# alevar/tiebrush

Measured on AMD Instinct MI355X. Metric: input alignment records/sec collapsed (tiebrush) + bases/sec covered (tiecov), higher is better.
Workload: dtype int64; 1 GPU; c3: 64 synthetic sorted BAMs x 5000000 100bp reads per GPU, --clip collapse + tiecov -c -j of the result; records_per_gpu=320000000, groups_out=25086541, parallelism=files-per-rank x1, ranks_seen=1, resident=SoA in HBM before the timed region, contexts=3

## Files before the change

### tiebrush_amd/csrc/collapse.hip

```cpp
#include <stdlib.h>

#include <chrono>

#include "cb_tiles.hpp"
#include "dev_common.hpp"
#include "rx_w64.hpp"
#include "scan_op.hpp"
#include "strategy.hpp"
#include "tbk_internal.h"
#include "wgroup.h"

namespace {

struct EffKey {
  uint32_t khi_h, khi_l;
  int32_t kend;
  uint32_t flag_cnt;
};
struct EffOp {
  __device__ __forceinline__ EffKey operator()(const EffKey& a, const EffKey& b) const {
    uint64_t ak = ((uint64_t)a.khi_h << 32) | a.khi_l, bk = ((uint64_t)b.khi_h << 32) | b.khi_l;
    bool take_b = (b.flag_cnt >> 31) || bk > ak || (bk == ak && b.kend > a.kend);
    EffKey r;
    r.khi_h = take_b ? b.khi_h : a.khi_h;
// ... 353 lines not shown
__global__ void col_recgroup_w_k(uint32_t n, const uint32_t* __restrict__ rec_sg, const uint32_t* __restrict__ ginv, int32_t* __restrict__ rec_group) {
  uint32_t i = blockIdx.x * blockDim.x + threadIdx.x;
  if (i >= n) return;
  const uint32_t sg = rec_sg[i];
  rec_group[i] = sg == 0xFFFFFFFFu ? -1 : (int32_t)ginv[sg];
}


constexpr uint32_t YS_NT = 1024;
constexpr uint32_t YS_NL = 128;
struct YsIn {
  uint32_t ng;
  const uint32_t* gperm;
  const uint32_t* ns;
  const uint32_t* gpoff;
  const uint16_t* pfile;
  const uint64_t* ghi;
  const uint64_t* gfmask;
};
__device__ __forceinline__ uint64_t ys_spread32(uint64_t x) {
  x = (x | (x << 16)) & 0x0000FFFF0000FFFFull;
  x = (x | (x << 8)) & 0x00FF00FF00FF00FFull;
  x = (x | (x << 4)) & 0x0F0F0F0F0F0F0F0Full;
  x = (x | (x << 2)) & 0x3333333333333333ull;
  x = (x | (x << 1)) & 0x5555555555555555ull;
  return x;
}
__device__ __forceinline__ void ys_mask_from_files(uint64_t files, uint32_t c, uint64_t* lo, uint64_t* hi) {
  const uint64_t a = ys_spread32(files & 0xFFFFFFFFull), b = ys_spread32(files >> 32);
  *lo = c == 0u ? a : (c == 1u ? a << 1 : (a | (a << 1)));
  *hi = c == 0u ? b : (c == 1u ? b << 1 : (b | (b << 1)));
}
__device__ __forceinline__ uint64_t wave_bit_transpose(uint64_t x) {
  const uint32_t lane = lane_id();
#define YS_TSTEP(J, M)                                                                     \
  {                                                                                        \
    const uint64_t tt = ((uint64_t)(uint32_t)__shfl_xor((int)(uint32_t)(x >> 32), J, 64) << 32) | (uint32_t)__shfl_xor((int)(uint32_t)x, J, 64); \
    x = (lane & J) ? (((tt >> J) & M) | (x & ~M)) : ((x & M) | ((tt & M) << J));           \
  }
  YS_TSTEP(32, 0x00000000FFFFFFFFull)
  YS_TSTEP(16, 0x0000FFFF0000FFFFull)
  YS_TSTEP(8, 0x00FF00FF00FF00FFull)
  YS_TSTEP(4, 0x0F0F0F0F0F0F0F0Full)
  YS_TSTEP(2, 0x3333333333333333ull)
  YS_TSTEP(1, 0x5555555555555555ull)
#undef YS_TSTEP
  return x;
}
struct YsAgg {
  uint32_t first_tid, last_tid;
  int32_t mx;
  uint32_t whole;
};
__device__ __forceinline__ YsAgg ys_combine(const YsAgg& a, const YsAgg& b) {
  if (b.last_tid == 0u) return a;
  if (a.last_tid == 0u) return b;
  YsAgg r;
  r.first_tid = a.first_tid;
  r.last_tid = b.last_tid;
  const bool joins = b.whole && b.first_tid == a.last_tid;
  r.mx = joins ? (a.mx > b.mx ? a.mx : b.mx) : b.mx;
  r.whole = joins ? a.whole : 0u;
  return r;
}
struct YsCells {
  uint32_t (*a)[YS_NL];
  uint32_t (*b)[YS_NL];
  int32_t (*m)[YS_NL];
  __device__ __forceinline__ YsAgg get(uint32_t x, uint32_t c) const { return YsAgg{a[x][c] & 0x7FFFFFFFu, b[x][c], m[x][c], a[x][c] >> 31}; }
  __device__ __forceinline__ void put(uint32_t x, uint32_t c, const YsAgg& v) const {
    a[x][c] = v.first_tid | (v.whole << 31);
    b[x][c] = v.last_tid;
    m[x][c] = v.mx;
  }
};
__device__ __forceinline__ YsAgg ys_chain_cells(const YsCells& P, uint32_t c, YsAgg run) {
  for (uint32_t x = 0; x < YS_NT / 64; ++x) {
    const YsAgg mine = P.get(x, c);
    P.put(x, c, run);
    run = ys_combine(run, mine);
  }
  return run;
}
__global__ __launch_bounds__(YS_NT) void yd_lcount_k(YsIn S, const uint4* __restrict__ gpk , uint32_t ntiles,
                                                     uint32_t* __restrict__ table , uint4* __restrict__ agg ,
                                                     uint64_t* __restrict__ gwb ) {
  __shared__ uint64_t wb[YS_NT / 64][YS_NL];
  __shared__ uint32_t g_tid[YS_NT];
  __shared__ int32_t g_e1[YS_NT];
  __shared__ uint32_t pa[YS_NT / 64][YS_NL], pb[YS_NT / 64][YS_NL];
  __shared__ int32_t pm[YS_NT / 64][YS_NL];
  const YsCells P{pa, pb, pm};
  uint64_t lo = 0, hi = 0;
  {
    const uint32_t o = blockIdx.x * YS_NT + threadIdx.x;
    if (o < S.ng) {
      const uint32_t sg = S.gperm[o];
      const uint32_t c = (uint32_t)S.ghi[sg] & 3u;
      const uint32_t n = S.gfmask ? 0u : S.ns[sg], p0 = S.gfmask ? 0u : S.gpoff[sg];
      uint64_t files = 0;
      if (S.gfmask)
        files = S.gfmask[sg];
      else
        for (uint32_t i = 0; i < n; ++i) files |= 1ull << S.pfile[p0 + i];
      ys_mask_from_files(files, c, &lo, &hi);
      const uint4 g = gpk[o];
      g_tid[threadIdx.x] = g.x;
      g_e1[threadIdx.x] = (int32_t)g.z + 1;
    }
  }
  {
    const uint32_t x = threadIdx.x >> 6, l = lane_id();
    const uint64_t a = wave_bit_transpose(lo), b = wave_bit_transpose(hi);
    wb[x][l] = a;
    wb[x][64u + l] = b;
    uint64_t* out = gwb + (size_t)blockIdx.x * (YS_NT / 64) * YS_NL + x * YS_NL;
    out[l] = a;
    out[64u + l] = b;
  }
  __syncthreads();
  for (uint32_t q = threadIdx.x; q < (YS_NT / 64) * YS_NL; q += YS_NT) {
    const uint32_t x = q / YS_NL, c = q % YS_NL;
    YsAgg A{0u, 0u, INT32_MIN, 1u};
    for (uint64_t m = wb[x][c]; m; m &= m - 1) {
      const uint32_t g = x * 64u + (uint32_t)__builtin_ctzll(m);
      A = ys_combine(A, YsAgg{g_tid[g], g_tid[g], g_e1[g], 1u});
    }
    P.put(x, c, A);
  }
  __syncthreads();
  if (threadIdx.x < YS_NL) {
    const uint32_t c = threadIdx.x;
    uint32_t n = 0;
    YsAgg A{0u, 0u, INT32_MIN, 1u};
    for (uint32_t x = 0; x < YS_NT / 64; ++x) {
      n += (uint32_t)__builtin_popcountll(wb[x][c]);
      A = ys_combine(A, P.get(x, c));
    }
    table[(size_t)c * ntiles + blockIdx.x] = n;
    agg[(size_t)c * ntiles + blockIdx.x] = make_uint4(A.first_tid, A.last_tid, (uint32_t)A.mx, A.whole);
  }
}
__global__ __launch_bounds__(256) void yd_lagg_scan_k(uint4* __restrict__ agg, uint32_t ntiles) {
  __shared__ uint4 part[256];
  uint4* row = agg + (size_t)blockIdx.x * ntiles;
  const uint32_t per = (ntiles + 255u) / 256u, i0 = threadIdx.x * per, i1 = i0 + per < ntiles ? i0 + per : ntiles;
  auto un = [](const uint4& v) { return YsAgg{v.x, v.y, (int32_t)v.z, v.w}; };
  auto pk = [](const YsAgg& a) { return make_uint4(a.first_tid, a.last_tid, (uint32_t)a.mx, a.whole); };
  YsAgg A{0u, 0u, INT32_MIN, 1u};
  for (uint32_t i = i0; i < i1; ++i) A = ys_combine(A, un(row[i]));
  part[threadIdx.x] = pk(A);
  __syncthreads();
  if (threadIdx.x == 0) {
    YsAgg run{0u, 0u, INT32_MIN, 1u};
    for (uint32_t q = 0; q < 256; ++q) {
      const YsAgg mine = un(part[q]);
      part[q] = pk(run);
      run = ys_combine(run, mine);
    }
  }
  __syncthreads();
  YsAgg run = un(part[threadIdx.x]);
  for (uint32_t i = i0; i < i1; ++i) {
    const YsAgg mine = un(row[i]);
    row[i] = pk(run);
    run = ys_combine(run, mine);
  }
}
__global__ __launch_bounds__(1024) void yd_lscan_k(uint32_t* __restrict__ table, uint32_t ntiles, uint64_t* __restrict__ totals,
                                                   unsigned long long* __restrict__ nit ) {
  __shared__ uint32_t sm[16];
  __shared__ uint32_t carry_s;
  uint32_t* row = table + (size_t)blockIdx.x * ntiles;
  constexpr uint32_t E = 8;
  if (threadIdx.x == 0) carry_s = 0;
  __syncthreads();
  for (uint32_t base = 0; base < ntiles; base += 1024 * E) {
    const uint32_t i0 = base + threadIdx.x * E;
    uint32_t v[E], s = 0;
#pragma unroll
    for (uint32_t e = 0; e < E; ++e) {
      v[e] = i0 + e < ntiles ? row[i0 + e] : 0u;
      s += v[e];
    }
    uint32_t tot;
    uint32_t ex = carry_s + block_excl_sum<uint32_t, 1024>(s, sm, &tot);
#pragma unroll
    for (uint32_t e = 0; e < E; ++e) {
      if (i0 + e < ntiles) row[i0 + e] = ex;
      ex += v[e];
    }
    __syncthreads();
    if (threadIdx.x == 0) carry_s += tot;
    __syncthreads();
  }
  if (threadIdx.x == 0) {
    totals[blockIdx.x] = carry_s;
    atomicAdd(nit, (unsigned long long)carry_s);
  }
}

struct YdWords {
  const uint64_t* w64;
// ... 43 lines not shown
    const uint32_t a = (h32 >> 20) & 0x3FFu, g = h32 & 0xFFFFFu;
    *e0 = st + a - 1u;
    *s1 = st + a + g;
    return 2u;
  }
  return 0u;
}

__global__ void yd_groups_k(ColIn I, uint32_t ng, const uint32_t* __restrict__ gperm, GroupAcc G, const uint64_t* __restrict__ shi,
                            const uint64_t* __restrict__ slo, YdGroups Q) {
  uint32_t o = blockIdx.x * blockDim.x + threadIdx.x;
  if (o >= ng) return;
  uint32_t sg = gperm[o];
  uint32_t q = G.first[sg];
  uint64_t h = shi[q], l = slo[q];
  int32_t st = (int32_t)(uint32_t)((h >> 2) & 0x7FFFFFFFull);
  const uint32_t tidp1 = (uint32_t)(h >> 33);
  const uint32_t en = (uint32_t)(st + (int32_t)(uint32_t)(l >> 32) - 1);
  uint32_t e0, s1;
  const uint32_t nk = yd_exons_from_key(l, (uint32_t)st, en, &e0, &s1);
  int nex = (int)nk;
  if (nex == 0) {
    const uint32_t r = (uint32_t)(G.rep[sg] & 0xFFFFFFFFull);
    walk_exons(I.pos[r], I.cig + I.cig_off[r], I.cig_off[r + 1] - I.cig_off[r], [](int, int) {}, &nex);
  }
  uint32_t xw = (uint32_t)nex;
  if (nk == 2u) {
    const uint32_t a = e0 - (uint32_t)st + 1u, g = s1 - e0 - 1u;
    if (a < (1u << 10) && g < (1u << 20)) xw = YD_X2 | (a << 20) | g;
  }
  Q.nex[o] = yd_nex_far(xw) ? (uint32_t)nex : 0u;
  Q.pk[o] = make_uint4(tidp1, (uint32_t)st, en, xw);
}

__global__ void yd_gexons_k(ColIn I, uint32_t ng, const uint32_t* __restrict__ gperm, GroupAcc G, const uint64_t* __restrict__ slo, YdGroups Q,
                            uint32_t* __restrict__ ex_s, uint32_t* __restrict__ ex_e) {
  uint32_t o = blockIdx.x * blockDim.x + threadIdx.x;
  if (o >= ng) return;
  const uint4 pk = Q.pk[o];
  if (!yd_nex_far(pk.w)) return;
  const uint32_t sg = gperm[o];
  uint32_t w = Q.xoff[o];
  {
    uint32_t e0, s1;
    const uint32_t nk = yd_exons_from_key(slo[G.first[sg]], pk.y, pk.z, &e0, &s1);
    if (nk) {
      ex_s[w] = pk.y;
      ex_e[w] = e0;
      if (nk == 2u) {
        ex_s[w + 1] = s1;
        ex_e[w + 1] = pk.z;
      }
      return;
    }
  }
  uint32_t r = (uint32_t)(G.rep[sg] & 0xFFFFFFFFull);
  int nex = 0;
  walk_exons(I.pos[r], I.cig + I.cig_off[r], I.cig_off[r + 1] - I.cig_off[r],
             [&](int es, int ee) {
               ex_s[w] = (uint32_t)es;
               ex_e[w] = (uint32_t)ee;
               ++w;
             },
             &nex);
}

struct YdEmit {
  YdGroups Q;
  YdItems Y;
  __device__ __forceinline__ void operator()(uint32_t t, uint64_t w) const {
    const uint32_t o = (uint32_t)w;
    const uint4 g = Q.pk[o];
    Y.pk[t] = make_uint4(g.x, g.y, g.z, Q.xoff[o]);
    Y.nex[t] = g.w;
  }
};

constexpr uint32_t YS_CAP = 15360;
constexpr uint32_t YS_NC = (YS_NT / 64) * YS_NL;
static_assert(YS_NC == 2 * YS_NT && YS_CAP >= 4 * YS_NC, "the staging array holds the cells' aggregates and counts first");
__global__ __launch_bounds__(YS_NT) void yd_lscatter_k(uint32_t ng, uint32_t ntiles, const uint32_t* __restrict__ table,
                                                       const uint64_t* __restrict__ totals, const uint4* __restrict__ agg,
                                                       const uint64_t* __restrict__ gwb , YdGroups Q,
                                                       YdItems Y, uint32_t* __restrict__ item) {
  __shared__ uint32_t off[YS_NL];
  __shared__ uint32_t pre[YS_NL + 1];
  __shared__ uint32_t lsum[YS_NL];
  __shared__ uint32_t lbase[YS_NL];
  __shared__ uint4 grec[YS_NT];
  __shared__ uint32_t stage[YS_CAP];
  const YsCells P{reinterpret_cast<uint32_t(*)[YS_NL]>(stage), reinterpret_cast<uint32_t(*)[YS_NL]>(stage + YS_NC),
                  reinterpret_cast<int32_t(*)[YS_NL]>(stage + 2 * YS_NC)};
  uint32_t(*pa)[YS_NL] = reinterpret_cast<uint32_t(*)[YS_NL]>(stage + 3 * YS_NC);
  const uint32_t t = threadIdx.x, c = t % YS_NL, x0 = t / YS_NL, x1 = x0 + YS_NT / YS_NL;
  const uint64_t* col = gwb + (size_t)blockIdx.x * YS_NC;
  const uint64_t m0 = col[t], m1 = col[YS_NT + t];
  if (t < YS_NL) lbase[t] = (uint32_t)totals[t];
  const uint32_t o = blockIdx.x * YS_NT + t;
  if (o < ng) grec[t] = Q.pk[o];
  __syncthreads();
  auto fold = [&](uint64_t m, uint32_t x) {
    pa[x][c] = (uint32_t)__builtin_popcountll(m);
    YsAgg A{0u, 0u, INT32_MIN, 1u};
    for (; m; m &= m - 1) {
      const uint4 g = grec[x * 64u + (uint32_t)__builtin_ctzll(m)];
      A = ys_combine(A, YsAgg{g.x, g.x, (int32_t)g.z + 1, 1u});
    }
    P.put(x, c, A);
  };
  fold(m0, x0);
  fold(m1, x1);
  __syncthreads();
  if (t < YS_NL) {
    const uint4 av = agg[(size_t)t * ntiles + blockIdx.x];
    (void)ys_chain_cells(P, t, YsAgg{av.x, av.y, (int32_t)av.z, av.w});
    uint32_t run = 0;
    for (uint32_t x = 0; x < YS_NT / 64; ++x) {
      const uint32_t n = pa[x][t];
      pa[x][t] = run;
      run += n;
    }
    lsum[t] = run;
  }
  __syncthreads();
  if (t < 64) {
    const uint32_t a = lsum[2 * t], b = lsum[2 * t + 1], inc = wave_incl_sum(a + b);
    const uint32_t ta = lbase[2 * t], tb = lbase[2 * t + 1], tinc = wave_incl_sum(ta + tb);
    pre[2 * t] = inc - a - b;
    pre[2 * t + 1] = inc - b;
    if (t == 63) pre[YS_NL] = inc;
    off[2 * t] = tinc - ta - tb + table[(size_t)(2 * t) * ntiles + blockIdx.x] - (inc - a - b);
    off[2 * t + 1] = tinc - tb + table[(size_t)(2 * t + 1) * ntiles + blockIdx.x] - (inc - b);
  }
  __syncthreads();
  const YsAgg A0 = P.get(x0, c), A1 = P.get(x1, c);
  const uint32_t s0 = pre[c] + pa[x0][c], s1 = pre[c] + pa[x1][c], T = pre[YS_NL];
  for (uint32_t r0 = 0; r0 < T; r0 += YS_CAP) {
    __syncthreads();
    const uint32_t r1 = r0 + YS_CAP;
    auto walk = [&](uint64_t m, uint32_t x, YsAgg A, uint32_t i) {
      if (i >= r1 || i + (uint32_t)__builtin_popcountll(m) <= r0) return;
      for (; m && i < r1; m &= m - 1, ++i) {
        const uint32_t g = x * 64u + (uint32_t)__builtin_ctzll(m);
        const uint4 v = grec[g];
        const bool head = A.last_tid == 0u || v.x != A.last_tid || (int32_t)v.y > A.mx;
        A = ys_combine(A, YsAgg{v.x, v.x, (int32_t)v.z + 1, 1u});
        if (i >= r0) stage[i - r0] = g | (c << 10) | ((uint32_t)head << 17);
      }
    };
    walk(m0, x0, A0, s0);
    walk(m1, x1, A1, s1);
    __syncthreads();
    const uint32_t n = T - r0 < YS_CAP ? T - r0 : YS_CAP;
    for (uint32_t i = t; i < n; i += YS_NT) {
      const uint32_t e = stage[i], g = e & (YS_NT - 1u), l = (e >> 10) & (YS_NL - 1u);
      const uint4 v = grec[g];
      const uint32_t pos = off[l] + r0 + i;
      Y.se[pos] = make_uint2(v.y, v.z);
      Y.nex[pos] = v.w | ((e >> 17) << 31);
      item[pos] = blockIdx.x * YS_NT + g;
    }
  }
}

struct SegMaxY {
  int32_t mx;
  uint32_t flag;
};
struct SegMaxYOp {
  __device__ __forceinline__ SegMaxY operator()(const SegMaxY& a, const SegMaxY& b) const {
    SegMaxY r;
    r.mx = b.flag ? b.mx : (a.mx > b.mx ? a.mx : b.mx);
    r.flag = a.flag | b.flag;
    return r;
  }
};
struct YdLoad {
  const uint64_t* list;
  YdItems Y;
  __device__ __forceinline__ bool list_head(uint32_t t) const {
    return t == 0 || (list[t] >> 32) != (list[t - 1] >> 32) || Y.tidp1(t) != Y.tidp1(t - 1);
  }
  __device__ __forceinline__ SegMaxY operator()(uint32_t t) const {
    SegMaxY s;
    s.mx = Y.end(t) + 1;
    s.flag = list_head(t) ? 1u : 0u;
    return s;
  }
};
struct HeadNex {
  uint32_t h, n;
};
struct HeadNexOp {
  __device__ __forceinline__ HeadNex operator()(const HeadNex& a, const HeadNex& b) const { return HeadNex{a.h + b.h, a.n + b.n}; }
};
struct YdAux {
  YdItems Y;
  __device__ __forceinline__ int2 operator()(uint32_t t) const { return make_int2(Y.start(t), (int)yd_nex_count(Y.nex[t])); }
};
struct YdHead {
  __device__ __forceinline__ HeadNex operator()(uint32_t, const SegMaxY& v, const SegMaxY&, const SegMaxY& ex, const int2& a) const {
    return HeadNex{(v.flag || a.x > ex.mx) ? 1u : 0u, (uint32_t)a.y};
  }
};
struct YdStore {
  YdItems Y;
  uint32_t *chain_first, *chain_noff;
  uint64_t* totals;
  uint32_t nit;
  __device__ __forceinline__ void operator()(uint32_t t, const SegMaxY&, const SegMaxY&, const SegMaxY&, const HeadNex& v, const HeadNex& ex,
                                             const int2&) const {
    if (v.h) {
      chain_first[ex.h] = t;
      chain_noff[ex.h] = ex.n;
    }
    if (t + 1 == nit) {
      totals[0] = ex.h + v.h;
      totals[1] = ex.n + v.n;
    }
  }
};

constexpr uint32_t YN_NT = 256, YN_ROWS = 4, YN_TILE = YN_NT * 4 * YN_ROWS;
__device__ __forceinline__ uint4 yn_load(const uint32_t* __restrict__ w, uint64_t i, uint32_t nit) {
  if (i + 3 < nit) return *reinterpret_cast<const uint4*>(w + i);
  uint4 v = make_uint4(0u, 0u, 0u, 0u);
  if (i < nit) v.x = w[i];
  if (i + 1 < nit) v.y = w[i + 1];
  if (i + 2 < nit) v.z = w[i + 2];
  return v;
}
__global__ __launch_bounds__(YN_NT) void yn_reduce_k(const uint32_t* __restrict__ w, uint32_t nit, unsigned long long* __restrict__ part) {
  __shared__ unsigned long long sm[YN_NT / 64];
  unsigned long long acc = 0;
#pragma unroll
  for (uint32_t r = 0; r < YN_ROWS; ++r) {
    const uint4 v = yn_load(w, (uint64_t)blockIdx.x * YN_TILE + ((uint64_t)r * YN_NT + threadIdx.x) * 4u, nit);
    const uint32_t h = (v.x >> 31) + (v.y >> 31) + (v.z >> 31) + (v.w >> 31);
    const uint32_t n = yd_nex_count(v.x) + yd_nex_count(v.y) + yd_nex_count(v.z) + yd_nex_count(v.w);
    acc += ((unsigned long long)h << 32) + n;
  }
  acc = wave_sum(acc);
// ... 809 lines not shown
      if (h32 == (0x80000000u | C_M)) shape = 0x80000000u;
      if ((h32 >> 30) == 3u) shape = h32;
    }
    g_key[2 * (size_t)o] = shi[q];
    g_key[2 * (size_t)o + 1] = (lo & 0xFFFFFFFF00000000ull) | shape;
  }
}
__global__ void col_recgroup_k(const uint64_t* __restrict__ pm, const uint32_t* __restrict__ val, const uint32_t* __restrict__ sgid,
                               const uint32_t* __restrict__ ginv, int32_t* __restrict__ rec_group) {
  const uint32_t m = (uint32_t)*pm;
  uint32_t q = blockIdx.x * blockDim.x + threadIdx.x;
  if (q < m) rec_group[val[q]] = (int32_t)ginv[sgid[q]];
}

__global__ void col_init_groups_k(const uint64_t* __restrict__ png, GroupAcc G, int32_t* __restrict__ g_yd) {
  const uint32_t ng = (uint32_t)*png;
  uint32_t g = blockIdx.x * blockDim.x + threadIdx.x;
  if (g >= ng) return;
  G.yc[g] = 0.0;
  G.ns[g] = 0;
  G.yxin[g] = 0;
  G.ydin[g] = 0;
  G.rep[g] = ~0ull;
  g_yd[g] = 0;
}

struct YdJob {
  ColIn I;
  uint32_t m, ng, cap;
  const uint32_t* val;
  const uint8_t* flags;
  const uint16_t* fidx;
  const uint32_t *sgid, *ginv, *gperm;
  GroupAcc G;
  const uint64_t *shi, *slo;
  int32_t* g_yd;
  int32_t* out_yd;
  bool win = false;
  uint32_t np = 0;
  const uint16_t* pfile = nullptr;
  const uint32_t *pgrp = nullptr, *gpoff = nullptr;
  const uint64_t* gfmask = nullptr;
};

}

int tbk_collapse_yd_run(tbk_ctx* ctx, void* jobp) {
  const YdJob J = *(const YdJob*)jobp;
  delete (YdJob*)jobp;
  const uint32_t B = 256;
  const uint32_t m = J.m, ng = J.ng;
  const ColIn& I = J.I;
  uint64_t* sc = ctx->d_scalars;
  TBK_HIP(hipSetDevice(ctx->device));
  const bool ph = ctx->dbg.phases;
  const auto p0 = std::chrono::steady_clock::now();
  auto p1 = p0, p2 = p0, p3 = p0;
  auto since = [](std::chrono::steady_clock::time_point a) { return std::chrono::duration<double, std::milli>(std::chrono::steady_clock::now() - a).count(); };
  TBK_HIP(hipMemsetAsync(sc, 0, 32 * sizeof(uint64_t), ctx->stream));
  {
    uint32_t *icnt = nullptr, *ioff = nullptr, *ocnt = nullptr, *ooff = nullptr;
    uint64_t nit64;
    const bool by_list = J.win && (!J.pgrp || tbk_yd_by_list(ctx, I.k));
    static_assert(YS_NL == 128, "tbk_yd_by_list (wgroup.h) knows the number of lists");
    const uint32_t ys_tiles = cdiv(ng, YS_NT);
    const YsIn S{ng, J.gperm, J.G.ns, J.gpoff, J.pfile, J.shi, J.gfmask};
    uint32_t* ys_table = nullptr;
    uint4* ys_agg = nullptr;
    uint64_t* ys_totals = nullptr;
    uint64_t* ys_wb = nullptr;
    uint32_t *yd_d = nullptr, *ys_item = nullptr;
    YdGroups Q{};
    if (by_list) {
      Q.pk = ws_alloc<uint4>(ctx, ng);
      Q.nex = ws_alloc<uint32_t>(ctx, ng);
      Q.xoff = ws_alloc<uint32_t>(ctx, ng);
      ys_table = ws_alloc<uint32_t>(ctx, (size_t)YS_NL * ys_tiles);
      ys_agg = ws_alloc<uint4>(ctx, (size_t)YS_NL * ys_tiles);
      ys_totals = ws_alloc<uint64_t>(ctx, YS_NL + 1);
      ys_wb = ws_alloc<uint64_t>(ctx, (size_t)ys_tiles * YS_NC);
      if (!Q.xoff || !ys_table || !ys_agg || !ys_totals || !ys_wb) return TBK_ENOMEM;
      TBK_LAUNCH(ctx, "yd_groups", yd_groups_k, cdiv(ng, B), B, 0, I, ng, J.gperm, J.G, J.shi, J.slo, Q);
      TBK_TRY(tbk_exscan_u32(ctx, Q.nex, Q.xoff, ng, sc + 5));
      TBK_LAUNCH(ctx, "yd_lcount", yd_lcount_k, ys_tiles, YS_NT, 0, S, Q.pk, ys_tiles, ys_table, ys_agg, ys_wb);
      TBK_LAUNCH(ctx, "yd_lscan", yd_lscan_k, YS_NL, 1024, 0, ys_table, ys_tiles, ys_totals, (unsigned long long*)(sc + 2));
      TBK_LAUNCH(ctx, "yd_lscan", yd_lagg_scan_k, YS_NL, 256, 0, ys_agg, ys_tiles);
    } else if (J.win) {
      ocnt = ws_alloc<uint32_t>(ctx, ng);
      ooff = ws_alloc<uint32_t>(ctx, ng);
      if (!ooff) return TBK_ENOMEM;
      TBK_LAUNCH(ctx, "yd_gcount", yd_gcount_w_k, cdiv(ng, B), B, 0, ng, J.gperm, J.G, J.shi, ocnt);
      TBK_TRY(tbk_exscan_u32(ctx, ocnt, ooff, ng, sc + 2));
    } else {
      icnt = ws_alloc<uint32_t>(ctx, m);
      ioff = ws_alloc<uint32_t>(ctx, m);
      if (!ioff) return TBK_ENOMEM;
      TBK_LAUNCH(ctx, "yd_count", yd_count_k, cdiv(m, B), B, 0, I, m, J.val, J.flags, J.fidx, icnt);
      TBK_TRY(tbk_exscan_u32(ctx, icnt, ioff, m, sc + 2));
    }
    TBK_HIP(hipMemcpyAsync(ctx->h_scalars, sc, 16 * sizeof(uint64_t), hipMemcpyDeviceToHost, ctx->stream));
    TBK_HIP(hipStreamSynchronize(ctx->stream));
    nit64 = ctx->h_scalars[2];
    p1 = p2 = p3 = std::chrono::steady_clock::now();
    if (nit64 >= (1ull << 32)) return TBK_E2BIG;
    const uint32_t nit = (uint32_t)nit64;
    if (nit) {
      uint64_t* iv = by_list ? nullptr : ws_alloc<uint64_t>(ctx, nit);
      uint64_t* iv2 = by_list ? nullptr : ws_alloc<uint64_t>(ctx, nit);
      uint32_t* io = by_list ? ws_alloc<uint32_t>(ctx, nit) : nullptr;
      yd_d = by_list ? ws_alloc<uint32_t>(ctx, nit) : nullptr;
      if (by_list && (!io || !yd_d)) return TBK_ENOMEM;
      ys_item = io;
      YdItems Y;
      if (by_list) {
        Y.pk = nullptr;
        Y.se = ws_alloc<uint2>(ctx, nit);
        Y.gxoff = Q.xoff;
        if (!Y.se) return TBK_ENOMEM;
      } else {
        Y.pk = ws_alloc<uint4>(ctx, nit);
      }
      Y.nex = ws_alloc<uint32_t>(ctx, nit);
      uint32_t* noff = ws_alloc<uint32_t>(ctx, nit);
      uint32_t* chain_first = ws_alloc<uint32_t>(ctx, nit);
      if (!chain_first) return TBK_ENOMEM;
      if (by_list) {
      } else if (J.win) {
        TBK_LAUNCH(ctx, "yd_fill", yd_fill_w_k, cdiv(J.np, B), B, 0, J.np, J.pfile, J.pgrp, J.gpoff, J.ginv, ooff, J.shi, iv);
      } else {
        ocnt = ws_alloc<uint32_t>(ctx, ng);
        ooff = ws_alloc<uint32_t>(ctx, ng);
        if (!ooff) return TBK_ENOMEM;
        TBK_LAUNCH(ctx, "yd_gcount", yd_gcount_k, cdiv(ng, B), B, 0, ng, m, J.gperm, J.G, ioff, icnt, ocnt);
        TBK_TRY(tbk_exscan_u32(ctx, ocnt, ooff, ng, nullptr));
        TBK_LAUNCH(ctx, "yd_fill", yd_fill_k, cdiv(m, B), B, 0, I, m, J.val, J.flags, J.fidx, J.sgid, J.ginv, ioff, ooff, J.G, iv);
      }
      if (!by_list) {
        Q.pk = ws_alloc<uint4>(ctx, ng);
        Q.nex = ws_alloc<uint32_t>(ctx, ng);
        Q.xoff = ws_alloc<uint32_t>(ctx, ng);
        if (!Q.xoff) return TBK_ENOMEM;
        TBK_LAUNCH(ctx, "yd_groups", yd_groups_k, cdiv(ng, B), B, 0, I, ng, J.gperm, J.G, J.shi, J.slo, Q);
        TBK_TRY(tbk_exscan_u32(ctx, Q.nex, Q.xoff, ng, sc + 5));
      }
      if (by_list) {
        TBK_LAUNCH(ctx, "yd_scatter", yd_lscatter_k, ys_tiles, YS_NT, 0, ng, ys_tiles, ys_table, ys_totals, ys_agg, ys_wb, Q, Y, io);
      } else {
        uint32_t bits = 1;
        while ((1ull << bits) < 2ull * I.k) ++bits;
        TBK_TRY(tbk_radix_sort_w64_emit(ctx, &iv, &iv2, nit, ((1ull << bits) - 1ull) << 32, true, YdEmit{Q, Y}, "yd_scatter"));
      }
      if (by_list) {
        const uint32_t ynb = cdiv(nit, YN_TILE);
        unsigned long long* ypart = ws_alloc<unsigned long long>(ctx, ynb);
        if (!ypart) return TBK_ENOMEM;
        TBK_LAUNCH(ctx, "yd_number", yn_reduce_k, ynb, YN_NT, 0, Y.nex, nit, ypart);
        TBK_LAUNCH(ctx, "yd_number", yn_spine_k, 1, 1024, 0, ypart, ynb, sc + 3);
        TBK_LAUNCH(ctx, "yd_number", yn_emit_k, ynb, YN_NT, 0, Y.nex, nit, ypart, chain_first, noff);
      } else {
        YdLoad ld{iv, Y};
        YdAux ax{Y};
        YdHead hd{};
        YdStore st{Y, chain_first, noff, sc + 3, nit};
        SegMaxY ident{INT32_MIN, 0u};
        TBK_TRY((scan_two_run<8, SegMaxY, SegMaxYOp, HeadNex, HeadNexOp, YdLoad, YdAux, YdHead, YdStore>(ctx, "yd_chains", nit, ld, ax, hd, st, SegMaxYOp{}, ident,
                                                                                              HeadNexOp{}, HeadNex{0u, 0u})));
      }
      TBK_HIP(hipMemcpyAsync(ctx->h_scalars, sc, 16 * sizeof(uint64_t), hipMemcpyDeviceToHost, ctx->stream));
      TBK_HIP(hipStreamSynchronize(ctx->stream));
      const uint32_t nchains = (uint32_t)ctx->h_scalars[3];
      const uint64_t nnodes = ctx->h_scalars[4], ngex = ctx->h_scalars[5];
      p2 = p3 = std::chrono::steady_clock::now();
      if (nnodes >= (1ull << 31)) return TBK_E2BIG;
      SegNodes N;
      N.s = ws_alloc<uint32_t>(ctx, nnodes + 1);
      N.e = ws_alloc<uint32_t>(ctx, nnodes + 1);
      N.nx = ws_alloc<int32_t>(ctx, nnodes + 1);
      uint32_t* ex_s = ws_alloc<uint32_t>(ctx, ngex + 1);
      uint32_t* ex_e = ws_alloc<uint32_t>(ctx, ngex + 1);
      uint32_t* ids_lane = ws_alloc<uint32_t>(ctx, nchains);
      uint32_t* ids_long = ws_alloc<uint32_t>(ctx, nchains);
      uint32_t* ids_over = ws_alloc<uint32_t>(ctx, nchains);
      uint32_t* bcnt = ws_alloc<uint32_t>(ctx, 4 * YD_NB + 4);
      if (!ids_over || !bcnt) return TBK_ENOMEM;
      uint32_t* bcur = bcnt + 2 * YD_NB;
      uint32_t* n_wave = bcur + 2 * YD_NB;
      uint32_t* n_over = n_wave + 1;
      TBK_HIP(hipMemsetAsync(bcnt, 0, (4 * YD_NB + 4) * sizeof(uint32_t), ctx->stream));
      TBK_LAUNCH(ctx, "yd_gexons", yd_gexons_k, cdiv(ng, B), B, 0, I, ng, J.gperm, J.G, J.slo, Q, ex_s, ex_e);
      const uint32_t wave_min = ctx->dbg.yd_wave_min ? ctx->dbg.yd_wave_min : YD_WAVE_MIN_DEFAULT;
      const uint32_t bgrid = ctx->dbg.yd_bgrid ? ctx->dbg.yd_bgrid : std::min(cdiv(nchains, B), YD_BGRID);
      TBK_LAUNCH(ctx, "yd_classify", yd_bucket_count_k, bgrid, B, 0, nchains, nit, wave_min, chain_first, bcnt);
      TBK_LAUNCH(ctx, "yd_classify", yd_bucket_off_k, 1, 1, 0, bcnt, bcur);
      TBK_LAUNCH(ctx, "yd_classify", yd_bucket_fill_k, bgrid, B, 0, nchains, nit, wave_min, chain_first, bcur, ids_lane, ids_long);
      uint32_t* hc = (uint32_t*)(ctx->h_scalars + 24);
      TBK_HIP(hipMemcpyAsync(hc, n_wave, sizeof(uint32_t), hipMemcpyDeviceToHost, ctx->stream));
      TBK_HIP(hipStreamSynchronize(ctx->stream));
      const uint32_t n_long = hc[0], n_lane = nchains - n_long;
      p3 = std::chrono::steady_clock::now();
      const bool literal = ctx->dbg.yd_literal;
      if (literal) {
        if (n_long) TBK_HIP(hipMemcpyAsync(ids_over, ids_long, (size_t)n_long * 4, hipMemcpyDeviceToDevice, ctx->stream));
        if (n_lane) TBK_HIP(hipMemcpyAsync(ids_over + n_long, ids_lane, (size_t)n_lane * 4, hipMemcpyDeviceToDevice, ctx->stream));
        hc[1] = nchains;
        TBK_HIP(hipMemcpyAsync(n_over, hc + 1, sizeof(uint32_t), hipMemcpyHostToDevice, ctx->stream));
        TBK_HIP(hipStreamSynchronize(ctx->stream));
      }
      hipStream_t aux = n_lane && n_long && !literal ? tbk_aux_stream(ctx) : nullptr;
      if (n_long && !literal) {
        hipStream_t keep = ctx->stream;
        if (aux) ctx->stream = aux;
        TBK_LAUNCH(ctx, "yd_wave", yd_wave_k, n_long, 64, 0, ids_long, n_wave, nchains, nit, chain_first, Y, YdWords{iv, io}, noff, ex_s, ex_e, J.g_yd,
                   yd_d, ids_over, n_over);
        ctx->stream = keep;
        if (aux) TBK_HIP(hipEventRecord(ctx->aux_done, aux));
      }
      if (n_lane && !literal)
        TBK_LAUNCH(ctx, "yd_lane", yd_lane_k<8>, cdiv(n_lane, 64), 64, 0, ids_lane, n_lane, nchains, nit, chain_first, Y, YdWords{iv, io}, ex_s, ex_e, J.g_yd,
                   yd_d, ids_over, n_over);
      if (n_long && aux) TBK_HIP(hipStreamWaitEvent(ctx->stream, ctx->aux_done, 0));
      TBK_LAUNCH(ctx, "yd_run_overflow", yd_run_k, cdiv(nchains, 64), 64, 0, ids_over, n_over, nchains, nit, chain_first, Y, YdWords{iv, io}, noff, ex_s, ex_e,
                 N, J.g_yd, yd_d);
    }
    if (by_list) {
      TBK_LAUNCH(ctx, "yd_gather", yd_lgather_k, ys_tiles, 512, 0, ng, ys_tiles, ys_table, ys_totals, yd_d, ys_item, J.gperm, J.G, J.cap, J.out_yd);
      TBK_HIP(hipStreamSynchronize(ctx->stream));
      if (ph)
        fprintf(stderr, "YD stage ms: counts %.1f | placement + numbering %.1f | buckets %.1f | list machines + gather %.1f (arena %.2f of %.2f GB, %zu overflow chunks)\n",
                std::chrono::duration<double, std::milli>(p1 - p0).count(), std::chrono::duration<double, std::milli>(p2 - p1).count(),
// ... 835 lines not shown
```

### tiebrush_amd/csrc/tbk_api.hip

```cpp
#include <sys/mman.h>

#include <algorithm>
#include <chrono>
#include <mutex>
#include <vector>
#include <new>

#include "tbk_internal.h"

namespace {
std::mutex g_reg_m;
struct RegEntry {
  void* p;
  int users;
};
std::vector<RegEntry> g_reg;
}

static void release_registered(tbk_ctx* ctx) {
  if (ctx->registered.empty()) return;
  (void)hipStreamSynchronize(ctx->stream);
  const auto r0 = std::chrono::steady_clock::now();
  struct RP {
    tbk_ctx* c;
// ... 365 lines not shown
      (void)hipStreamDestroy(ctx->aux);
      ctx->aux = nullptr;
    }
  }
  return ctx->aux;
}

tbk_ctx* tbk_side_ctx(tbk_ctx* ctx) {
  if (!ctx->side_ctx && tbk_create(ctx->device, &ctx->side_ctx) != 0) ctx->side_ctx = nullptr;
  if (ctx->side_ctx) {
    ctx->side_ctx->profiling = ctx->profiling;
    ctx->side_ctx->dbg = ctx->dbg;
  }
  return ctx->side_ctx;
}
int tbk_side_begin(tbk_ctx* side, size_t arena_hint) {
  if (hipSetDevice(side->device) != hipSuccess) return TBK_EHIP;
  tbk_prof_begin_call(side);
  return ws_begin_call(side, arena_hint);
}
void tbk_side_end(tbk_ctx* side) { tbk_prof_end_call(side); }

static void merge_side_times(tbk_ctx* ctx) {
  if (!ctx->side_times_pending || !ctx->side_ctx) return;
  ctx->side_times_pending = false;
  for (auto& t : ctx->side_ctx->last_times) {
    bool found = false;
    for (auto& u : ctx->last_times)
      if (strcmp(u.name, t.name) == 0) {
        u.ms += t.ms;
        u.launches += t.launches;
        found = true;
        break;
      }
    if (!found) ctx->last_times.push_back(t);
  }
}

static int yd_stage_on(tbk_ctx* run_on, void* job, size_t hint) {
  if (hipSetDevice(run_on->device) != hipSuccess) return TBK_EHIP;
  tbk_prof_begin_call(run_on);
  int rc = ws_begin_call(run_on, hint);
  if (rc == 0) rc = tbk_collapse_yd_run(run_on, job);
  tbk_prof_end_call(run_on);
  return rc;
}

static int finish_yd(tbk_ctx* ctx) {
  if (!ctx->yd_pending) return 0;
  ctx->yd_worker->wait();
  ctx->yd_pending = false;
  ctx->ws_base_off = 0;
  if (ctx->yd_ctx) {
    ctx->last_times = ctx->yd_ctx->last_times;
    if (ctx->yd_rc != 0) ctx->last_error = ctx->yd_ctx->last_error;
  }
  return ctx->yd_rc;
}

void tbk_debug_parse(const char* spec, TbkDebug* out) {
  *out = TbkDebug();
  if (!spec) return;
  std::string s(spec);
  size_t at = 0;
  while (at < s.size()) {
    size_t end = s.find(',', at);
    if (end == std::string::npos) end = s.size();
    const std::string kv = s.substr(at, end - at);
    at = end + 1;
    const size_t eq = kv.find('=');
    const std::string k = kv.substr(0, eq), v = eq == std::string::npos ? std::string("1") : kv.substr(eq + 1);
    const unsigned long long u = strtoull(v.c_str(), nullptr, 0);
    const bool on = v != "0";
    if (k == "path") out->path = v == "sort" ? 1 : (v == "window" ? 2 : 0);
    else if (k == "raw") out->raw = on ? 1 : 0;
    else if (k == "sort") out->sort = v == "radix" ? 1 : (v == "runs" ? 2 : 0);
    else if (k == "scan") out->scan = v == "lookback" ? 1 : (v == "3pass" ? 2 : 0);
    else if (k == "hash_mask") out->hash_mask = (uint32_t)u;
    else if (k == "qhash_mask") out->qhash_mask = u;
    else if (k == "yd_wave_min") out->yd_wave_min = (uint32_t)u;
    else if (k == "yd_bgrid") out->yd_bgrid = (uint32_t)u;
    else if (k == "yd_radix") out->yd_radix = on;
    else if (k == "yd_literal") out->yd_literal = on;
    else if (k == "yd_own_arena") out->yd_own_arena = on;
    else if (k == "wg_dense_verify") out->wg_dense_verify = on;
    else if (k == "wg_rank_merge") out->wg_rank_merge = on;
    else if (k == "cov_legacy") out->cov_legacy = on;
    else if (k == "cov_bundle_scan") out->cov_bundle_scan = on;
    else if (k == "cov_prep") out->cov_prep = on;
    else if (k == "cov_tile_cap") out->cov_tile_cap = u;
    else if (k == "junc_radix") out->junc_radix = on;
    else if (k == "no_junc_agg") out->no_junc_agg = on;
    else if (k == "jh_cap") out->jh_cap = (uint32_t)u;
    else if (k == "index_chain") out->index_chain = on;
    else if (k == "no_register") out->no_register = on;
    else if (k == "phases") out->phases = on;
    else if (k == "no_bounce") out->no_bounce = on;
    else if (k == "fmt_slice") out->fmt_slice = u;
  }
}

extern "C" {

int tbk_abi_version(void) { return TBK_ABI_VERSION; }

int tbk_set_debug(tbk_ctx* ctx, const char* spec) {
  if (!ctx) return TBK_EINVAL;
  tbk_debug_parse(spec, &ctx->dbg);
  if (ctx->yd_ctx) ctx->yd_ctx->dbg = ctx->dbg;
  if (ctx->side_ctx) ctx->side_ctx->dbg = ctx->dbg;
  return 0;
}

const char* tbk_strerror(int s) {
  switch (s) {
    case TBK_OK: return "ok";
    case TBK_EINVAL: return "invalid argument";
    case TBK_ENOMEM: return "out of memory";
    case TBK_EHIP: return "HIP runtime error";
    case TBK_E2BIG: return "output capacity too small";
    case TBK_EUNSUPPORTED: return "option or input outside the supported/pinned semantics";
    case TBK_EUNSORTED: return "input not coordinate-sorted";
    case TBK_EFATALOP: return "unknown opcode (tiecov accepts only M/I/D/N/S)";
    case TBK_ECOLLISION: return "key hash collision survived all reseeds";
    case TBK_ENODEVICE: return "no usable gfx950 device";
  }
  return "unknown status";
}

int tbk_create(int device_ordinal, tbk_ctx** out) {
  if (!out) return TBK_EINVAL;
  *out = nullptr;
  int ndev = 0;
  if (hipGetDeviceCount(&ndev) != hipSuccess || ndev <= 0 || device_ordinal < 0 || device_ordinal >= ndev) return TBK_ENODEVICE;
  tbk_ctx* ctx = new (std::nothrow) tbk_ctx();
  if (!ctx) return TBK_ENOMEM;
  ctx->device = device_ordinal;
  tbk_debug_parse(getenv("TBK_DEBUG"), &ctx->dbg);
  bool ok = hipSetDevice(device_ordinal) == hipSuccess;
  hipDeviceProp_t prop;
  if (ok && hipGetDeviceProperties(&prop, device_ordinal) == hipSuccess) ctx->num_cu = prop.multiProcessorCount;
  ok = ok && hipStreamCreateWithFlags(&ctx->own_stream, hipStreamNonBlocking) == hipSuccess;
  ctx->stream = ctx->own_stream;
  ok = ok && hipMalloc((void**)&ctx->d_scalars, 64 * sizeof(uint64_t)) == hipSuccess;
  if (ok) ctx->d_err = (uint32_t*)(ctx->d_scalars + 15);
  ok = ok && hipHostMalloc((void**)&ctx->h_scalars, (64 + 4096) * sizeof(uint64_t), hipHostMallocDefault) == hipSuccess;
  if (!ok) {
    tbk_destroy(ctx);
    return TBK_EHIP;
  }
  *out = ctx;
  return 0;
}

int tbk_collapse_finish_yd(tbk_ctx* ctx) {
  if (!ctx) return TBK_EINVAL;
  return finish_yd(ctx);
}

void tbk_destroy(tbk_ctx* ctx) {
  if (!ctx) return;
  (void)finish_yd(ctx);
  tbk_bam_release(ctx);
  delete ctx->yd_worker;
  ctx->yd_worker = nullptr;
  delete ctx->side_worker;
// ... 444 lines not shown
```

### tiebrush_amd/csrc/tbk_internal.h

```cpp
#pragma once
#include <hip/hip_runtime.h>
#include <stdint.h>
#include <stdio.h>
#include <string.h>

#include <string>
#include <condition_variable>
#include <functional>
#include <mutex>
#include <thread>
#include <utility>
#include <vector>

#include "../../include/tbk.h"

enum : uint32_t {
  TBK_DERR_UNSORTED = 1u << 0,
  TBK_DERR_COLLISION = 1u << 1,
  TBK_DERR_FATALOP = 1u << 2,
  TBK_DERR_SPAN = 1u << 3,
  TBK_DERR_NCIGAR = 1u << 4,
  TBK_DERR_FRACTIONAL = 1u << 5,
  TBK_DERR_OVERFLOW = 1u << 6,
  TBK_DERR_INTERNAL = 1u << 7,
  TBK_DERR_BIGBUCKET = 1u << 8,
  TBK_DERR_RAWORDER = 1u << 9
};

struct KTime {
  const char* name;
  hipEvent_t a, b;
};

struct TbkWorker {
  std::thread th;
  std::mutex m;
  std::condition_variable cv;
  std::function<void()> job;
  bool busy = false, quit = false, started = false;
  void post(std::function<void()> j) {
    {
      std::lock_guard<std::mutex> lk(m);
      if (!started) {
        started = true;
        th = std::thread([this]() {
          std::unique_lock<std::mutex> lk2(m);
          for (;;) {
            cv.wait(lk2, [&] { return quit || (bool)job; });
            if (quit) return;
            std::function<void()> run = std::move(job);
            job = nullptr;
            lk2.unlock();
            run();
            lk2.lock();
            busy = false;
            cv.notify_all();
          }
        });
      }
      job = std::move(j);
      busy = true;
    }
    cv.notify_all();
  }
  void wait() {
    std::unique_lock<std::mutex> lk(m);
    cv.wait(lk, [&] { return !busy; });
  }
  ~TbkWorker() {
    {
      std::lock_guard<std::mutex> lk(m);
      quit = true;
    }
    cv.notify_all();
    if (th.joinable()) th.join();
  }
};

struct TbkDebug {
  int path = 0;
  int raw = -1;
  int sort = 0;
  int scan = 0;
  uint32_t hash_mask = 0xFFFFFFFFu;
  uint64_t qhash_mask = ~0ull;
  uint32_t yd_wave_min = 0;
  uint32_t yd_bgrid = 0;
  bool yd_radix = false;
  bool yd_literal = false;
  bool yd_own_arena = false;
  bool wg_dense_verify = false, wg_rank_merge = false;
  bool cov_legacy = false, cov_bundle_scan = false, cov_prep = false, junc_radix = false, no_junc_agg = false;
  uint64_t cov_tile_cap = 0;
  uint32_t jh_cap = 0;
  bool index_chain = false;
  bool no_register = false;
  bool no_bounce = false;
  bool phases = false;
  uint64_t fmt_slice = 0;
};
void tbk_debug_parse(const char* spec, TbkDebug* out);

struct tbk_ctx {
  int device = 0;
  TbkDebug dbg;
  hipStream_t own_stream = nullptr;
  hipStream_t stream = nullptr;
  hipStream_t aux = nullptr;
  hipEvent_t aux_done = nullptr;
  char* ws = nullptr;
  size_t ws_cap = 0, ws_off = 0;
  size_t ws_top = 0;
  bool ws_top_mode = false;
  bool ws_borrowed = false;
  std::vector<std::pair<char*, size_t>> ws_overflow;
  size_t ws_over_used = 0;
  uint32_t* d_err = nullptr;
  uint64_t* d_scalars = nullptr;
  uint64_t* h_scalars = nullptr;
  hipEvent_t stage_ev = nullptr;
  char* d_view = nullptr;
  size_t d_view_cap = 0;
  struct ViewPrep {
    bool valid = false;
    const void* cig = nullptr;
    uint32_t n = 0;
    int32_t *start = nullptr, *end = nullptr, *yi = nullptr;
    uint32_t *jcnt = nullptr, *ridx = nullptr;
    const void* agg = nullptr;
    uint32_t agg_tiles = 0;
    uint64_t n_bases = 0, sum_abs = 0, n_junc = 0;
    uint32_t err = 0;
  } view_prep;
  bool profiling = false;
  std::vector<KTime> ktimes;
  std::vector<hipEvent_t> ev_pool;
  size_t ev_used = 0;
  std::vector<tbk_kernel_time> last_times;
  std::string last_error;
  int num_cu = 256;
  void* yd_job = nullptr;
  tbk_ctx* yd_ctx = nullptr;
  TbkWorker* yd_worker = nullptr;
  bool yd_pending = false;
  int yd_rc = 0;
  size_t ws_base_off = 0;
  tbk_ctx* side_ctx = nullptr;
  TbkWorker* side_worker = nullptr;
  bool side_times_pending = false;
  std::vector<void*> registered;
  char* d_unpack = nullptr;
  size_t d_unpack_cap = 0;
  std::vector<uint8_t> unpack_tbm;
  void* bam_dev = nullptr;
  void* enc = nullptr;
  void* ix = nullptr;
  void* stager = nullptr;
  char* bounce = nullptr;
  char* kept = nullptr;
  size_t kept_cap = 0;
  uint32_t kept_n = 0;
  uint32_t* kept_rep = nullptr;
  double* kept_yc = nullptr;
  int64_t* kept_yx = nullptr;
  int32_t* kept_yd = nullptr;
  char* d_names = nullptr;
  uint64_t* d_name_off = nullptr;
  uint32_t n_names = 0;
  void* fmt_pin[2] = {nullptr, nullptr};
  size_t fmt_pin_cap = 0;
};
// ... 103 lines not shown
```

Measured before the change: 20.55 billion records/s.

## Add single-target fast path to list count and scatter kernels

When every group in a tile shares one target id, the count kernel skips the general per-cell aggregate chaining and uses shared-memory atomics for per-list max end and counts. The scatter kernel transposes the masks so each row of lanes scans one list with DPP row shifts. It also splits the packed group record into padded SoA shared arrays to cut bank conflicts. This removes the general combine logic for the common sorted case, but adds branch divergence and more shared memory, and the correctness of the DPP-based prefix has to match the general path.

```diff
diff --git a/tiebrush_amd/csrc/collapse.hip b/tiebrush_amd/csrc/collapse.hip
--- a/tiebrush_amd/csrc/collapse.hip
+++ b/tiebrush_amd/csrc/collapse.hip
@@ -459,10 +459,24 @@
   }
   return run;
 }
+__device__ __forceinline__ uint32_t ys_one_tid(const uint4* __restrict__ gpk, uint32_t ng, uint32_t general) {
+  const uint32_t o0 = blockIdx.x * YS_NT, o1 = (ng - o0 < YS_NT ? ng : o0 + YS_NT) - 1u;
+  const uint32_t a = gpk[o0].x, b = gpk[o1].x;
+  return !general && a == b ? a : 0u;
+}
+#define YS_ROW_SHR(v, N, idle) __builtin_amdgcn_update_dpp((int)(idle), (int)(v), 0x110 + (N), 0xf, 0xf, false)
 __global__ __launch_bounds__(YS_NT) void yd_lcount_k(YsIn S, const uint4* __restrict__ gpk , uint32_t ntiles,
                                                      uint32_t* __restrict__ table , uint4* __restrict__ agg ,
-                                                     uint64_t* __restrict__ gwb ) {
+                                                     uint64_t* __restrict__ gwb ,
+                                                     uint32_t general ) {
   __shared__ uint64_t wb[YS_NT / 64][YS_NL];
+  __shared__ int32_t lmx[YS_NL];
+  __shared__ uint32_t lnn[YS_NL];
+  const uint32_t tid1 = ys_one_tid(gpk, S.ng, general);
+  if (threadIdx.x < YS_NL) {
+    lmx[threadIdx.x] = INT32_MIN;
+    lnn[threadIdx.x] = 0u;
+  }
   __shared__ uint32_t g_tid[YS_NT];
   __shared__ int32_t g_e1[YS_NT];
   __shared__ uint32_t pa[YS_NT / 64][YS_NL], pb[YS_NT / 64][YS_NL];
@@ -496,6 +510,25 @@
     out[64u + l] = b;
   }
   __syncthreads();
+  if (tid1) {
+    const uint32_t c = threadIdx.x % YS_NL, x0 = threadIdx.x / YS_NL, x1 = x0 + YS_NT / YS_NL;
+    const uint64_t m0 = wb[x0][c], m1 = wb[x1][c];
+    int32_t mx = INT32_MIN;
+    for (uint64_t m = m0; m; m &= m - 1) mx = max(mx, g_e1[x0 * 64u + (uint32_t)__builtin_ctzll(m)]);
+    for (uint64_t m = m1; m; m &= m - 1) mx = max(mx, g_e1[x1 * 64u + (uint32_t)__builtin_ctzll(m)]);
+    if (m0 | m1) {
+      atomicMax(&lmx[c], mx);
+      atomicAdd(&lnn[c], (uint32_t)(__builtin_popcountll(m0) + __builtin_popcountll(m1)));
+    }
+    __syncthreads();
+    if (threadIdx.x < YS_NL) {
+      const uint32_t n = lnn[threadIdx.x];
+      table[(size_t)threadIdx.x * ntiles + blockIdx.x] = n;
+      agg[(size_t)threadIdx.x * ntiles + blockIdx.x] =
+          n ? make_uint4(tid1, tid1, (uint32_t)lmx[threadIdx.x], 1u) : make_uint4(0u, 0u, (uint32_t)INT32_MIN, 1u);
+    }
+    return;
+  }
   for (uint32_t q = threadIdx.x; q < (YS_NT / 64) * YS_NL; q += YS_NT) {
     const uint32_t x = q / YS_NL, c = q % YS_NL;
     YsAgg A{0u, 0u, INT32_MIN, 1u};
@@ -705,36 +738,85 @@
 __global__ __launch_bounds__(YS_NT) void yd_lscatter_k(uint32_t ng, uint32_t ntiles, const uint32_t* __restrict__ table,
                                                        const uint64_t* __restrict__ totals, const uint4* __restrict__ agg,
                                                        const uint64_t* __restrict__ gwb , YdGroups Q,
-                                                       YdItems Y, uint32_t* __restrict__ item) {
+                                                       YdItems Y, uint32_t* __restrict__ item, uint32_t general ) {
   __shared__ uint32_t off[YS_NL];
   __shared__ uint32_t pre[YS_NL + 1];
   __shared__ uint32_t lsum[YS_NL];
   __shared__ uint32_t lbase[YS_NL];
-  __shared__ uint4 grec[YS_NT];
+  constexpr uint32_t YS_NS = YS_NT + YS_NT / 64;
+  __shared__ uint32_t g_tid[YS_NS], g_st[YS_NS], g_en[YS_NS], g_xw[YS_NS];
+  auto slot = [](uint32_t g) { return g + (g >> 6); };
   __shared__ uint32_t stage[YS_CAP];
   const YsCells P{reinterpret_cast<uint32_t(*)[YS_NL]>(stage), reinterpret_cast<uint32_t(*)[YS_NL]>(stage + YS_NC),
                   reinterpret_cast<int32_t(*)[YS_NL]>(stage + 2 * YS_NC)};
   uint32_t(*pa)[YS_NL] = reinterpret_cast<uint32_t(*)[YS_NL]>(stage + 3 * YS_NC);
   const uint32_t t = threadIdx.x, c = t % YS_NL, x0 = t / YS_NL, x1 = x0 + YS_NT / YS_NL;
   const uint64_t* col = gwb + (size_t)blockIdx.x * YS_NC;
-  const uint64_t m0 = col[t], m1 = col[YS_NT + t];
+  uint64_t m0 = col[t], m1 = col[YS_NT + t];
   if (t < YS_NL) lbase[t] = (uint32_t)totals[t];
   const uint32_t o = blockIdx.x * YS_NT + t;
-  if (o < ng) grec[t] = Q.pk[o];
+  const uint32_t tid1 = ys_one_tid(Q.pk, ng, general);
+  const uint32_t rx = t % (YS_NT / 64), rl0 = t / (YS_NT / 64), rl1 = rl0 + YS_NL / 2;
+  constexpr uint32_t YS_RS = YS_NT / 64 + 1;
+  uint64_t* tw = reinterpret_cast<uint64_t*>(stage);
+  static_assert(2 * YS_NL * YS_RS <= YS_CAP, "the columns fit the staging array");
+  if (o < ng) {
+    const uint4 g = Q.pk[o];
+    g_tid[slot(t)] = g.x;
+    g_st[slot(t)] = g.y;
+    g_en[slot(t)] = g.z;
+    g_xw[slot(t)] = g.w;
+  }
+  if (tid1) {
+    tw[c * YS_RS + x0] = m0;
+    tw[c * YS_RS + x1] = m1;
+  }
   __syncthreads();
+  int32_t b0 = INT32_MIN, b1 = INT32_MIN;
+  uint32_t q0 = 0, q1 = 0;
+  if (tid1) {
+    m0 = tw[rl0 * YS_RS + rx];
+    m1 = tw[rl1 * YS_RS + rx];
+    auto fold1 = [&](uint64_t m) {
+      if (!m) return INT32_MIN;
+      int32_t v = INT32_MIN;
+      for (; m; m &= m - 1) v = max(v, (int32_t)g_en[rx * 65u + (uint32_t)__builtin_ctzll(m)]);
+      return v + 1;
+    };
+    int32_t v0 = fold1(m0), v1 = fold1(m1);
+    uint32_t n0 = (uint32_t)__builtin_popcountll(m0), n1 = (uint32_t)__builtin_popcountll(m1);
+#define YS_SCAN_STEP(N)                                 \
+  v0 = max(v0, YS_ROW_SHR(v0, N, INT32_MIN));           \
+  v1 = max(v1, YS_ROW_SHR(v1, N, INT32_MIN));           \
+  n0 += (uint32_t)YS_ROW_SHR(n0, N, 0);                 \
+  n1 += (uint32_t)YS_ROW_SHR(n1, N, 0);
+    YS_SCAN_STEP(1) YS_SCAN_STEP(2) YS_SCAN_STEP(4) YS_SCAN_STEP(8)
+#undef YS_SCAN_STEP
+    if (rx == YS_NT / 64 - 1u) {
+      lsum[rl0] = n0;
+      lsum[rl1] = n1;
+    }
+    const uint4 a0 = agg[(size_t)rl0 * ntiles + blockIdx.x], a1 = agg[(size_t)rl1 * ntiles + blockIdx.x];
+    b0 = max(a0.y == tid1 ? (int32_t)a0.z : INT32_MIN, YS_ROW_SHR(v0, 1, INT32_MIN));
+    b1 = max(a1.y == tid1 ? (int32_t)a1.z : INT32_MIN, YS_ROW_SHR(v1, 1, INT32_MIN));
+    q0 = (uint32_t)YS_ROW_SHR(n0, 1, 0);
+    q1 = (uint32_t)YS_ROW_SHR(n1, 1, 0);
+  }
   auto fold = [&](uint64_t m, uint32_t x) {
     pa[x][c] = (uint32_t)__builtin_popcountll(m);
     YsAgg A{0u, 0u, INT32_MIN, 1u};
     for (; m; m &= m - 1) {
-      const uint4 g = grec[x * 64u + (uint32_t)__builtin_ctzll(m)];
-      A = ys_combine(A, YsAgg{g.x, g.x, (int32_t)g.z + 1, 1u});
+      const uint32_t gs = x * 65u + (uint32_t)__builtin_ctzll(m);
+      A = ys_combine(A, YsAgg{g_tid[gs], g_tid[gs], (int32_t)g_en[gs] + 1, 1u});
     }
     P.put(x, c, A);
   };
-  fold(m0, x0);
-  fold(m1, x1);
+  if (!tid1) {
+    fold(m0, x0);
+    fold(m1, x1);
+  }
   __syncthreads();
-  if (t < YS_NL) {
+  if (!tid1 && t < YS_NL) {
     const uint4 av = agg[(size_t)t * ntiles + blockIdx.x];
     (void)ys_chain_cells(P, t, YsAgg{av.x, av.y, (int32_t)av.z, av.w});
     uint32_t run = 0;
@@ -756,8 +838,9 @@
     off[2 * t + 1] = tinc - tb + table[(size_t)(2 * t + 1) * ntiles + blockIdx.x] - (inc - b);
   }
   __syncthreads();
-  const YsAgg A0 = P.get(x0, c), A1 = P.get(x1, c);
-  const uint32_t s0 = pre[c] + pa[x0][c], s1 = pre[c] + pa[x1][c], T = pre[YS_NL];
+  YsAgg A0{0u, 0u, INT32_MIN, 1u}, A1 = A0;
+  if (!tid1) A0 = P.get(x0, c), A1 = P.get(x1, c);
+  const uint32_t s0 = tid1 ? pre[rl0] + q0 : pre[c] + pa[x0][c], s1 = tid1 ? pre[rl1] + q1 : pre[c] + pa[x1][c], T = pre[YS_NL];
   for (uint32_t r0 = 0; r0 < T; r0 += YS_CAP) {
     __syncthreads();
     const uint32_t r1 = r0 + YS_CAP;
@@ -765,22 +848,36 @@
       if (i >= r1 || i + (uint32_t)__builtin_popcountll(m) <= r0) return;
       for (; m && i < r1; m &= m - 1, ++i) {
         const uint32_t g = x * 64u + (uint32_t)__builtin_ctzll(m);
-        const uint4 v = grec[g];
-        const bool head = A.last_tid == 0u || v.x != A.last_tid || (int32_t)v.y > A.mx;
-        A = ys_combine(A, YsAgg{v.x, v.x, (int32_t)v.z + 1, 1u});
+        const uint32_t gs = slot(g), vx = g_tid[gs];
+        const bool head = A.last_tid == 0u || vx != A.last_tid || (int32_t)g_st[gs] > A.mx;
+        A = ys_combine(A, YsAgg{vx, vx, (int32_t)g_en[gs] + 1, 1u});
         if (i >= r0) stage[i - r0] = g | (c << 10) | ((uint32_t)head << 17);
       }
     };
-    walk(m0, x0, A0, s0);
-    walk(m1, x1, A1, s1);
+    auto walk1 = [&](uint64_t m, uint32_t l, int32_t mx, uint32_t i) {
+      if (i >= r1 || i + (uint32_t)__builtin_popcountll(m) <= r0) return;
+      for (; m && i < r1; m &= m - 1, ++i) {
+        const uint32_t bit = (uint32_t)__builtin_ctzll(m), g = rx * 64u + bit;
+        const int32_t st = (int32_t)g_st[rx * 65u + bit], en1 = (int32_t)g_en[rx * 65u + bit] + 1;
+        const bool head = st > mx;
+        mx = max(mx, en1);
+        if (i >= r0) stage[i - r0] = g | (l << 10) | ((uint32_t)head << 17);
+      }
+    };
+    if (tid1) {
+      walk1(m0, rl0, b0, s0);
+      walk1(m1, rl1, b1, s1);
+    } else {
+      walk(m0, x0, A0, s0);
+      walk(m1, x1, A1, s1);
+    }
     __syncthreads();
     const uint32_t n = T - r0 < YS_CAP ? T - r0 : YS_CAP;
     for (uint32_t i = t; i < n; i += YS_NT) {
       const uint32_t e = stage[i], g = e & (YS_NT - 1u), l = (e >> 10) & (YS_NL - 1u);
-      const uint4 v = grec[g];
-      const uint32_t pos = off[l] + r0 + i;
-      Y.se[pos] = make_uint2(v.y, v.z);
-      Y.nex[pos] = v.w | ((e >> 17) << 31);
+      const uint32_t gs = slot(g), pos = off[l] + r0 + i;
+      Y.se[pos] = make_uint2(g_st[gs], g_en[gs]);
+      Y.nex[pos] = g_xw[gs] | ((e >> 17) << 31);
       item[pos] = blockIdx.x * YS_NT + g;
     }
   }
@@ -1756,7 +1853,7 @@
       if (!Q.xoff || !ys_table || !ys_agg || !ys_totals || !ys_wb) return TBK_ENOMEM;
       TBK_LAUNCH(ctx, "yd_groups", yd_groups_k, cdiv(ng, B), B, 0, I, ng, J.gperm, J.G, J.shi, J.slo, Q);
       TBK_TRY(tbk_exscan_u32(ctx, Q.nex, Q.xoff, ng, sc + 5));
-      TBK_LAUNCH(ctx, "yd_lcount", yd_lcount_k, ys_tiles, YS_NT, 0, S, Q.pk, ys_tiles, ys_table, ys_agg, ys_wb);
+      TBK_LAUNCH(ctx, "yd_lcount", yd_lcount_k, ys_tiles, YS_NT, 0, S, Q.pk, ys_tiles, ys_table, ys_agg, ys_wb, ctx->dbg.yd_general ? 1u : 0u);
       TBK_LAUNCH(ctx, "yd_lscan", yd_lscan_k, YS_NL, 1024, 0, ys_table, ys_tiles, ys_totals, (unsigned long long*)(sc + 2));
       TBK_LAUNCH(ctx, "yd_lscan", yd_lagg_scan_k, YS_NL, 256, 0, ys_agg, ys_tiles);
     } else if (J.win) {
@@ -1818,7 +1915,8 @@
         TBK_TRY(tbk_exscan_u32(ctx, Q.nex, Q.xoff, ng, sc + 5));
       }
       if (by_list) {
-        TBK_LAUNCH(ctx, "yd_scatter", yd_lscatter_k, ys_tiles, YS_NT, 0, ng, ys_tiles, ys_table, ys_totals, ys_agg, ys_wb, Q, Y, io);
+        TBK_LAUNCH(ctx, "yd_scatter", yd_lscatter_k, ys_tiles, YS_NT, 0, ng, ys_tiles, ys_table, ys_totals, ys_agg, ys_wb, Q, Y, io,
+                   ctx->dbg.yd_general ? 1u : 0u);
       } else {
         uint32_t bits = 1;
         while ((1ull << bits) < 2ull * I.k) ++bits;
diff --git a/tiebrush_amd/csrc/tbk_api.hip b/tiebrush_amd/csrc/tbk_api.hip
--- a/tiebrush_amd/csrc/tbk_api.hip
+++ b/tiebrush_amd/csrc/tbk_api.hip
@@ -471,6 +471,7 @@
     else if (k == "yd_bgrid") out->yd_bgrid = (uint32_t)u;
     else if (k == "yd_radix") out->yd_radix = on;
     else if (k == "yd_literal") out->yd_literal = on;
+    else if (k == "yd_general") out->yd_general = on;
     else if (k == "yd_own_arena") out->yd_own_arena = on;
     else if (k == "wg_dense_verify") out->wg_dense_verify = on;
     else if (k == "wg_rank_merge") out->wg_rank_merge = on;
diff --git a/tiebrush_amd/csrc/tbk_internal.h b/tiebrush_amd/csrc/tbk_internal.h
--- a/tiebrush_amd/csrc/tbk_internal.h
+++ b/tiebrush_amd/csrc/tbk_internal.h
@@ -87,6 +87,7 @@
   uint32_t yd_wave_min = 0;
   uint32_t yd_bgrid = 0;
   bool yd_radix = false;
+  bool yd_general = false;
   bool yd_literal = false;
   bool yd_own_arena = false;
   bool wg_dense_verify = false, wg_rank_merge = false;
```

Result: no change. 20.47 billion records/s (-0.4%).
